# schmeing/ReSeq

Measured on AMD Instinct MI355X. Metric: simulated read-pairs/sec (2x150 bp), higher is better.
Workload: dtype f64

## Files before the change

### reseq_amd/csrc/rsq_format.h

```cpp
#pragma once
#include "rsq_reads.h"

namespace rsq {

#if RSQ_DEVICE_BUILD
#ifndef RSQ_BIN_KEYS_LDS
#define RSQ_BIN_KEYS_LDS 4096
#endif
constexpr uint32_t kBinKeysLds = RSQ_BIN_KEYS_LDS;
constexpr uint32_t kBinItemsPerThread = 16, kBinBlock = 256;

__device__ inline void bin_count_key(uint32_t key, bool valid, uint32_t n_keys, uint32_t *hist, uint32_t *s_hist) {
    if (n_keys <= kBinKeysLds) {
        for (uint32_t k = threadIdx.x; k < n_keys; k += blockDim.x) s_hist[k] = 0;
        __syncthreads();
        if (valid) atomicAdd(&s_hist[key], 1u);
        __syncthreads();
        for (uint32_t k = threadIdx.x; k < n_keys; k += blockDim.x)
            if (s_hist[k]) atomicAdd(&hist[k], s_hist[k]);
    } else if (valid) atomicAdd(&hist[key], 1u);
}
__global__ void __launch_bounds__(kBinBlock) k_pair_tiles(DevSim S, const Fragment *frags, const FragmentVar *fvars, uint64_t n_pairs, uint64_t adapter_only_first, uint16_t *key_of,
                                                         uint32_t *hist) {
    __shared__ uint32_t s_hist[kBinKeysLds];
    const uint64_t pair = (uint64_t)blockIdx.x * blockDim.x + threadIdx.x;
    const bool valid = pair < n_pairs;
    uint32_t key = 0;
    if (valid) {
        Fragment f{};
        if (frags) f = frags[pair];
        const PairStream ps = pair_stream(frags ? &f : nullptr, fvars ? fvars[pair].sub : 0u, adapter_only_first + pair);
        key = draw_tile(S, ps.c0, ps.c1, ps.c2, pair_c3(kDomPair, ps.strand, 2, f.allele));
        key_of[pair] = (uint16_t)key;
    }
    bin_count_key(key, valid, S.n_tiles, hist, s_hist);
}
__global__ void __launch_bounds__(kBinBlock) k_record_tiles(DevSim S, const uint8_t *segs, uint64_t first_index, uint64_t n, uint16_t *key_of, uint32_t *hist) {
    __shared__ uint32_t s_hist[kBinKeysLds];
    const uint64_t i = (uint64_t)blockIdx.x * blockDim.x + threadIdx.x;
    const bool valid = i < n;
    uint32_t key = 0;
    if (valid) {
        const uint64_t idx = first_index + i;
        key = (segs[i] ? S.n_tiles : 0u) + draw_tile(S, (uint32_t)idx, (uint32_t)(idx >> 32), 0u, pair_c3(kDomErrModel, 0, 2));
        key_of[i] = (uint16_t)key;
    }
    bin_count_key(key, valid, 2u * S.n_tiles, hist, s_hist);
}
__global__ void __launch_bounds__(1024) k_bins_plan(const uint32_t *hist, uint32_t n_keys, uint32_t n_bins, uint32_t *bin_first, uint32_t *bin_count, uint32_t *cursor,
                                                    uint32_t *chunk_ptr, uint32_t *next_chunk, uint32_t *workers) {
    __shared__ uint32_t s_part[1024], s_chunks[1024];
    const uint32_t t = threadIdx.x, per = (n_bins + 1023u) / 1024u, lo = t * per < n_bins ? t * per : n_bins, hi = lo + per < n_bins ? lo + per : n_bins;
    uint32_t items = 0, chunks = 0;
    for (uint32_t b = lo; b < hi; ++b) {
        const uint32_t c = hist[b % n_keys];
        if (b < n_keys) items += c;
        chunks += (c + 63u) / 64u;
    }
    s_part[t] = items;
    s_chunks[t] = chunks;
    __syncthreads();
    for (uint32_t d = 1; d < 1024u; d <<= 1) {
        const uint32_t a = t >= d ? s_part[t - d] : 0u, c = t >= d ? s_chunks[t - d] : 0u;
        __syncthreads();
        s_part[t] += a;
        s_chunks[t] += c;
        __syncthreads();
    }
    uint32_t at = s_part[t] - items, chunk_at = s_chunks[t] - chunks;
    for (uint32_t b = lo; b < hi; ++b) {
        const uint32_t c = hist[b % n_keys];
        if (b < n_keys) {
            cursor[b] = at;
            for (uint32_t r = b; r < n_bins; r += n_keys) bin_first[r] = at, bin_count[r] = c;
            at += c;
        }
        chunk_ptr[b] = chunk_at;
        chunk_at += (c + 63u) / 64u;
        next_chunk[b] = workers[b] = 0;
    }
    if (t == 1023u) chunk_ptr[n_bins] = s_chunks[1023];
}
__global__ void __launch_bounds__(kBinBlock) k_bin_scatter(const uint16_t *key_of, uint64_t n, uint32_t n_keys, uint32_t *cursor, uint32_t *perm, const Fragment *frags,
                                                          const FragmentVar *fvars, Fragment *frags_sorted, FragmentVar *fvars_sorted) {
    __shared__ uint32_t s_count[kBinKeysLds], s_base[kBinKeysLds];
    const uint64_t first = (uint64_t)blockIdx.x * (kBinBlock * kBinItemsPerThread);
    auto place = [&](uint32_t at, uint64_t i) {
        perm[at] = (uint32_t)i;
        if (frags) frags_sorted[at] = frags[i];
        if (fvars) fvars_sorted[at] = fvars[i];
    };
    if (n_keys > kBinKeysLds) {
        for (uint32_t j = 0; j < kBinItemsPerThread; ++j) {
            const uint64_t i = first + (uint64_t)j * kBinBlock + threadIdx.x;
            if (i < n) place(atomicAdd(&cursor[key_of[i]], 1u), i);
        }
        return;
    }
    for (uint32_t k = threadIdx.x; k < n_keys; k += kBinBlock) s_count[k] = 0;
    __syncthreads();
    uint32_t rank[kBinItemsPerThread], key[kBinItemsPerThread];
#pragma unroll
    for (uint32_t j = 0; j < kBinItemsPerThread; ++j) {
        const uint64_t i = first + (uint64_t)j * kBinBlock + threadIdx.x;
        key[j] = i < n ? key_of[i] : 0xFFFFFFFFu;
        rank[j] = i < n ? atomicAdd(&s_count[key[j]], 1u) : 0u;
    }
    __syncthreads();
    for (uint32_t k = threadIdx.x; k < n_keys; k += kBinBlock)
        if (s_count[k]) s_base[k] = atomicAdd(&cursor[k], s_count[k]);
    __syncthreads();
#pragma unroll
    for (uint32_t j = 0; j < kBinItemsPerThread; ++j)
        if (key[j] != 0xFFFFFFFFu) place(s_base[key[j]] + rank[j], first + (uint64_t)j * kBinBlock + threadIdx.x);
}

struct FragmentRange {
    uint32_t lo[2], hi[2];
};
__global__ void k_fragment_range(const uint8_t *segs, const uint32_t *frag_len, uint64_t n, FragmentRange range, uint32_t *first_bad) {
    const uint64_t i = (uint64_t)blockIdx.x * blockDim.x + threadIdx.x;
    if (i >= n) return;
    const uint32_t seg = segs[i] ? 1u : 0u, fl = frag_len[i];
    if (fl < range.lo[seg] || fl >= range.hi[seg]) atomicMin(first_bad, (uint32_t)i);
}
__global__ void k_record_flags(const uint8_t *segs, uint64_t n, uint32_t *flags) {
    const uint64_t i = (uint64_t)blockIdx.x * blockDim.x + threadIdx.x;
    if (i < n) flags[i] = segs[i] ? 1u : 0u;
}
__global__ void k_record_partition(const uint8_t *segs, uint64_t n, const uint64_t *ones_before, uint32_t *rec_index, uint32_t *rec_count) {
    const uint64_t i = (uint64_t)blockIdx.x * blockDim.x + threadIdx.x;
    const uint32_t n1 = (uint32_t)ones_before[n], n0 = (uint32_t)n - n1;
    if (i == 0) {
        rec_count[0] = n0;
        rec_count[1] = n1;
    }
    if (i >= n) return;
    const uint32_t before = (uint32_t)ones_before[i];
    if (segs[i]) rec_index[n0 + before] = (uint32_t)i;
    else rec_index[(uint32_t)i - before] = (uint32_t)i;
}

__global__ void __launch_bounds__(256) k_methylation_templates(DevSim S, const Fragment *frags, uint64_t n_pairs, RawLayout raw) {
    const uint64_t r = (uint64_t)blockIdx.x * blockDim.x + threadIdx.x;
    if (r >= 2u * n_pairs) return;
    const uint32_t seg = r >= n_pairs ? 1u : 0u;
    convert_template(S, frags[r - seg * n_pairs], seg, raw.templates + r * raw.template_words, raw.template_words);
}

__global__ void __launch_bounds__(256) k_variant_templates(DevSim S, const Fragment *frags, const FragmentVar *fvars, uint64_t n_pairs, RawLayout raw) {
    const uint64_t r = (uint64_t)blockIdx.x * blockDim.x + threadIdx.x;
    if (r >= 2u * n_pairs) return;
    const uint32_t seg = r >= n_pairs ? 1u : 0u;
    const uint64_t pair = r - seg * n_pairs;
    variant_template(S, frags[pair], fvars[pair], seg, raw.templates + r * raw.template_words, raw.template_words);
}

template <bool PERM, uint32_t ITEMS>
struct WaveImage {
    const uint64_t *offsets;
    char *dst;
    uint32_t lane, skew, bytes, slot_at;
    uint64_t row, item, g_begin;
    bool active, through_lds;
    static __device__ __forceinline__ uint64_t first() { return (uint64_t)blockIdx.x * ITEMS; }
    __device__ __forceinline__ WaveImage(const uint64_t *offsets, uint64_t n, char *dst, uint32_t lds_bytes, const uint32_t *perm, uint32_t lane) : offsets(offsets), dst(dst), lane(lane) {
        const uint64_t last = first() + ITEMS < n ? first() + ITEMS : n;
        row = first() + (lane & (ITEMS - 1u));
        active = row < last;
        item = PERM ? (active ? perm[row] : 0u) : row;
        g_begin = PERM ? (active ? offsets[item] : 0u) : offsets[first()];
        const uint64_t g_end = PERM ? (active ? offsets[item + 1u] : 0u) : offsets[last];
        skew = (uint32_t)((uint64_t)(uintptr_t)(dst + g_begin) & 15u);
        bytes = (uint32_t)(g_end - g_begin);
        const uint32_t slot = (lds_bytes / ITEMS) & ~15u;
        through_lds = PERM ? __all(skew + bytes <= slot) != 0 : skew + bytes <= lds_bytes;
        slot_at = PERM ? (lane & (ITEMS - 1u)) * slot : 0u;
    }
    __device__ __forceinline__ RSQ_LDS char *item_text(char *image) const { return (RSQ_LDS char *)image + slot_at + skew + (PERM ? 0u : (uint32_t)(offsets[item] - g_begin)); }
    __device__ __forceinline__ void store_out(const char *image) const {
        __syncthreads();
        const uint32_t lo = skew, hi = skew + bytes;
        char *g_chunk0 = dst + g_begin - skew;
        const char *s_from = image + slot_at;
        for (uint32_t c = (PERM ? lane / ITEMS : lane) * 16u; c < hi; c += (PERM ? 64u / ITEMS : 64u) * 16u) {
            if (c >= lo && c + 16u <= hi) {
                *reinterpret_cast<uint4 *>(g_chunk0 + c) = *reinterpret_cast<const uint4 *>(s_from + c);
            } else {
                for (uint32_t b = c < lo ? lo : c; b < c + 16u && b < hi; ++b) g_chunk0[b] = s_from[b];
            }
        }
    }
};

#ifndef RSQ_FORMAT_RECORDS
#define RSQ_FORMAT_RECORDS 16
#endif
constexpr uint32_t kFormatRecords = RSQ_FORMAT_RECORDS, kFormatLdsMax = 16u * 1024u, kFormatLdsMin = 1024u;
RSQ_HD uint32_t format_lds_bytes(uint64_t record_bytes, bool slots) {
    const uint64_t want = (kFormatRecords * record_bytes + 16u + 127u) & ~(uint64_t)127u;
    const uint32_t image = (uint32_t)(want < kFormatLdsMin ? kFormatLdsMin : want > kFormatLdsMax ? kFormatLdsMax : want);
    return !slots ? image : image + 16u * kFormatRecords < kFormatLdsMax ? image + 16u * kFormatRecords : kFormatLdsMax;
}
__global__ void __launch_bounds__(256) k_max_size(const uint32_t *sizes, uint64_t n, uint32_t *longest) {
    uint32_t m = 0;
    for (uint64_t i = (uint64_t)blockIdx.x * blockDim.x + threadIdx.x; i < n; i += (uint64_t)gridDim.x * blockDim.x) m = max(m, sizes[i]);
    for (uint32_t d = 32; d; d >>= 1) m = max(m, (uint32_t)__shfl_xor((int)m, (int)d, 64));
    if ((threadIdx.x & 63u) == 0 && m) atomicMax(longest, m);
}
template <bool PERM>
__global__ void __launch_bounds__(64) k_format_write(DevSim S, NameTable names, const Fragment *frags, uint64_t n_pairs, uint64_t adapter_only_first, RawLayout raw,
                                                    const uint64_t *offsets0, const uint64_t *offsets1, char *dst0, char *dst1, uint64_t cap0, uint64_t cap1,
                                                    const FragmentVar *fvars, const uint32_t *perm, uint32_t lds_bytes) {
    extern __shared__ __attribute__((aligned(16))) char s_text[];
    using Image = WaveImage<PERM, kFormatRecords>;
    const uint32_t lane = threadIdx.x, seg = blockIdx.y, part = lane / kFormatRecords;
    constexpr uint32_t kLineParts = 32u / kFormatRecords;
    const bool is_qual = part >= kLineParts;
    const uint32_t sub = part % kLineParts;
    if (Image::first() >= n_pairs) return;
    const uint64_t *offsets = seg ? offsets1 : offsets0;
    char *dst = seg ? dst1 : dst0;
    if (offsets[n_pairs] > (seg ? cap1 : cap0)) return;
    const Image im(offsets, n_pairs, dst, lds_bytes, perm, lane);
    const uint64_t pair = im.item;
    ReadMeta m;
    Fragment f;
    FragmentVar fv;
    uint64_t r = 0;
    if (im.active) {
        r = (uint64_t)seg * n_pairs + im.row;
        m = raw.meta[r];
        if (frags) f = frags[pair];
        if (frags && fvars) fv = fvars[pair];
    }
    const WordColumn seq = raw.seq_of(r), qual = raw.qual_of(r), ops = raw.ops_of(r);
    const uint64_t ao_number = adapter_only_first + pair + 1u;
    if (!im.through_lds) {
        if (im.active && part == 0u) format_record(S, names, frags != nullptr, f, ao_number, m, seq, qual, ops, dst + offsets[pair], frags && fvars, fv);
        return;
    }
    if (im.active) {
        const uint32_t header = (uint32_t)(offsets[pair + 1u] - offsets[pair]) - 2u * m.read_len - 4u;
        const uint32_t all_words = (m.read_len + 3u) >> 2, per = (all_words + kLineParts - 1u) / kLineParts;
        const uint32_t first_word = sub * per, line_at = header + (is_qual ? m.read_len + 3u : 0u);
        const uint32_t part_at = part == 0u ? 0u : line_at + (4u * first_word < m.read_len ? 4u * first_word : m.read_len);
        WordSinkT<RSQ_LDS char *> t(im.item_text(s_text) + part_at);
        if (part == 0u) format_header(S, names, frags != nullptr, f, ao_number, m, ops, t, frags && fvars, fv);
        format_line_part(is_qual ? qual : seq, m.read_len, is_qual, first_word, per, sub == kLineParts - 1u, t);
        t.finish();
    }
    im.store_out(s_text);
}

RSQ_HD uint32_t error_model_record_size(const ReadMeta &m, uint32_t id_len) { return 1u + id_len + 1u + m.cigar_chars + 2u + digits_u32(m.num_errors) + 1u + 2u * m.read_len + 4u; }
struct RecordIds {
    const char *chars;
    const uint64_t *off;
    const uint32_t *at, *len;
    RSQ_HD const char *begin(uint64_t i) const { return chars + (off ? off[i] : (uint64_t)at[i] + 1u); }
    RSQ_HD uint32_t length(uint64_t i) const { return off ? (uint32_t)(off[i + 1] - off[i]) : len[i]; }
};
__global__ void __launch_bounds__(256) k_record_text_sizes(RawLayout raw, uint64_t n, RecordIds ids, uint32_t *sizes) {
    const uint64_t row = (uint64_t)blockIdx.x * blockDim.x + threadIdx.x;
    if (row >= n) return;
    const uint64_t i = raw.item_of(row);
    sizes[i] = error_model_record_size(raw.meta[row], ids.length(i));
}
template <bool PERM>
__global__ void __launch_bounds__(64) k_record_text_waves(RawLayout raw, uint64_t n, RecordIds ids, const uint64_t *offsets, char *dst, uint64_t cap, uint32_t lds_bytes) {
    extern __shared__ __attribute__((aligned(16))) char s_text[];
    using Image = WaveImage<PERM, kFormatRecords>;
    constexpr uint32_t kLineParts = 32u / kFormatRecords;
    const uint32_t lane = threadIdx.x, part = lane / kFormatRecords, sub = part % kLineParts;
    const bool is_qual = part >= kLineParts;
    if (Image::first() >= n || offsets[n] > cap) return;
    const Image im(offsets, n, dst, lds_bytes, raw.order, lane);
    const uint64_t row = im.row, item = im.item;
    const bool active = im.active;
    ReadMeta m{};
    if (active) m = raw.meta[row];
    const WordColumn seq = raw.seq_of(active ? row : 0u), qual = raw.qual_of(active ? row : 0u), ops = raw.ops_of(active ? row : 0u);
    auto header = [&](auto &t) {
        t.ch('@');
        t.str(ids.begin(item), ids.length(item));
        t.ch(' ');
        cigar_replay(ops, m, t);
        t.str(" E", 2);
        t.num((uint32_t)m.num_errors);
        t.ch('\n');
    };
    if (!im.through_lds) {
        if (active && part == 0u) {
            WordSinkT<char *> t(dst + offsets[item]);
            header(t);
            format_line(seq, m.read_len, false, t);
            format_line(qual, m.read_len, true, t);
            t.finish();
        }
        return;
    }
    if (active) {
        const uint32_t head = (uint32_t)(offsets[item + 1u] - offsets[item]) - 2u * m.read_len - 4u;
        const uint32_t all_words = (m.read_len + 3u) >> 2, per = (all_words + kLineParts - 1u) / kLineParts, first_word = sub * per;
        const uint32_t line_at = head + (is_qual ? m.read_len + 3u : 0u), part_at = part == 0u ? 0u : line_at + (4u * first_word < m.read_len ? 4u * first_word : m.read_len);
        WordSinkT<RSQ_LDS char *> t(im.item_text(s_text) + part_at);
        if (part == 0u) header(t);
        format_line_part(is_qual ? qual : seq, m.read_len, is_qual, first_word, per, sub == kLineParts - 1u, t);
        t.finish();
    }
    im.store_out(s_text);
}

#endif

}
```

### reseq_amd/csrc/rsq_sam.h

```cpp
#pragma once
#include "rsq_format.h"

namespace rsq {

struct SamMate {
    uint16_t q, t;
    uint16_t lead, trail;
    uint16_t cigar_chars;
    uint16_t pad;
    uint32_t bytes;
};
static_assert(sizeof(SamMate) == 16, "two mates are one 32-byte load");
struct SamPair {
    SamMate mate[2];
};

RSQ_HD uint32_t sam_op_at(const WordColumn &ops, uint32_t it) { return (ops.at(it >> 4) >> ((it & 15u) * 2u)) & 3u; }

RSQ_HD SamMate sam_walk(const WordColumn &ops, const ReadMeta &m) {
    SamMate w{};
    const uint32_t n = m.n_iter_m;
    uint32_t chars = 0;
    if (m.plain) {
        w.q = w.t = (uint16_t)n;
        if (n) chars = digits_u32(n) + 1u;
    } else {
        uint32_t q = 0, t = 0, run = 0, cur = 3u, runs = 0;
        auto flush = [&](bool last) {
            if (!run) return;
            if (cur == 1u && runs == 1u) w.lead = (uint16_t)run;
            else if (cur == 1u && last) w.trail = (uint16_t)run;
            else chars += digits_u32(run) + 1u;
        };
        for (uint32_t it = 0; it < n; ++it) {
            if (!(it & 15u) && it + 16u <= n && !ops.at(it >> 4)) {
                if (cur != 0u) {
                    flush(false);
                    cur = 0u;
                    run = 0;
                    ++runs;
                }
                run += 16u;
                q += 16u;
                t += 16u;
                it += 15u;
                continue;
            }
            const uint32_t c = sam_op_at(ops, it);
            if (c != cur) {
                flush(false);
                cur = c;
                run = 0;
                ++runs;
            }
            ++run;
            q += c != 1u;
            t += c != 2u;
        }
        flush(true);
        w.q = (uint16_t)q;
        w.t = (uint16_t)t;
    }
    const uint32_t clip = (uint32_t)m.read_len - w.q;
    if (clip) chars += digits_u32(clip) + 1u;
    w.cigar_chars = (uint16_t)(chars ? chars : 1u);
    return w;
}

template <class Sink>
RSQ_HD void sam_cigar(const WordColumn &ops, const ReadMeta &m, const SamMate &w, bool reverse, Sink &t) {
    const uint32_t clip = (uint32_t)m.read_len - w.q;
    bool any = false;
    if (reverse && clip) {
        t.element('S', clip);
        any = true;
    }
    if (m.plain) {
        if (m.n_iter_m) {
            t.element('M', m.n_iter_m);
            any = true;
        }
    } else {
        const uint32_t lo = w.lead, hi = (uint32_t)m.n_iter_m - w.trail;
        uint32_t cur = 3u, run = 0;
        for (uint32_t i = lo; i < hi; ++i) {
            const uint32_t it = reverse ? hi - 1u - (i - lo) : i;
            if ((reverse ? (it & 15u) == 15u && it >= lo + 15u : !(it & 15u) && it + 16u <= hi) && (cur == 0u || !run) && !ops.at(it >> 4)) {
                cur = 0u;
                run += 16u;
                i += 15u;
                continue;
            }
            const uint32_t c = sam_op_at(ops, it);
            if (c != cur) {
                if (run) t.element(cur == 0u ? 'M' : cur == 1u ? 'D' : 'I', run);
                cur = c;
                run = 0;
            }
            ++run;
        }
        if (run) {
            t.element(cur == 0u ? 'M' : cur == 1u ? 'D' : 'I', run);
            any = true;
        }
    }
    if (!reverse && clip) {
        t.element('S', clip);
        any = true;
    }
    if (!any) t.ch('*');
}

struct SamAlign {
    uint32_t flag, pos, pnext;
    int32_t tlen;
    uint32_t mapped, reverse;
};
RSQ_HD SamAlign sam_align(bool has_f, const Fragment &f, uint32_t seg, const SamMate &w0, const SamMate &w1) {
    SamAlign a{};
    if (!has_f || !f.len) {
        a.flag = seg ? 141u : 77u;
        return a;
    }
    const uint32_t end = f.start + f.len;
    int32_t pos[2], last[2];
    for (uint32_t s = 0; s < 2u; ++s) {
        const SamMate &w = s ? w1 : w0;
        const bool rev = s != f.strand;
        const uint32_t d_left = rev ? w.trail : w.lead, d_right = rev ? w.lead : w.trail;
        pos[s] = (int32_t)((rev ? end - w.t : f.start) + 1u + d_left);
        last[s] = pos[s] + (int32_t)((uint32_t)w.t - d_left - d_right) - 1;
    }
    const uint32_t o = seg ^ 1u;
    const bool rev = seg != f.strand;
    a.mapped = 1u;
    a.reverse = rev ? 1u : 0u;
    a.flag = 0x1u | 0x2u | (rev ? 0x10u : 0x20u) | (seg ? 0x80u : 0x40u);
    a.pos = (uint32_t)pos[seg];
    a.pnext = (uint32_t)pos[o];
    const int32_t span = (last[0] > last[1] ? last[0] : last[1]) - (pos[0] < pos[1] ? pos[0] : pos[1]) + 1;
    const bool leftmost = pos[seg] < pos[o] || (pos[seg] == pos[o] && seg == 0u);
    a.tlen = leftmost ? span : -span;
    return a;
}

template <class Sink>
RSQ_HD void sam_qname(const DevSim &S, const NameTable &names, bool has_f, const Fragment &f, uint64_t adapter_only_number, const ReadMeta &m, Sink &t) {
    t.str(names.base_identifier, names.base_len);
    if (has_f) {
        const uint32_t end = f.start + f.len;
        t.num(f.block);
        t.ch('_');
        t.num(f.number);
        t.ch(':');
        t.num(f.strand ? end : f.start + 1u);
        t.ch(':');
        t.str(names.names + names.name_ptr[f.seq], names.name_ptr[f.seq + 1] - names.name_ptr[f.seq]);
        t.ch(':');
        t.num(f.strand ? f.start + 1u : end);
    } else {
        t.ch('0');
        t.ch('_');
        t.num(adapter_only_number);
        t.str(":0:Adapter:0", 12);
    }
    t.ch(':');
    t.num((uint32_t)S.tiles[m.tile_id]);
    t.str(":1337:1337", 10);
}
RSQ_HD uint32_t sam_qname_size(const DevSim &S, const NameTable &names, bool has_f, const Fragment &f, uint64_t adapter_only_number, const ReadMeta &m) {
    uint32_t n = names.base_len + 1u + digits_u32(S.tiles[m.tile_id]) + 10u;
    if (has_f) {
        const uint32_t end = f.start + f.len;
        n += digits_u32(f.block) + 1u + digits_u32(f.number) + 1u + digits_u32(f.start + 1u) + 1u + (names.name_ptr[f.seq + 1] - names.name_ptr[f.seq]) + 1u + digits_u32(end);
    } else n += 2u + digits_u64(adapter_only_number) + 12u;
    return n;
}
RSQ_HD uint32_t sam_tlen_chars(int32_t v) { return v < 0 ? 1u + digits_u32((uint32_t)-(int64_t)v) : digits_u32((uint32_t)v); }

template <class Sink>
RSQ_HD void sam_head(const DevSim &S, const NameTable &names, bool has_f, const Fragment &f, uint64_t adapter_only_number, const ReadMeta &m, const WordColumn &ops, const SamMate &w,
                     const SamAlign &a, Sink &t) {
    sam_qname(S, names, has_f, f, adapter_only_number, m, t);
    t.ch('\t');
    t.num(a.flag);
    t.ch('\t');
    if (a.mapped) {
        t.str(names.names + names.name_ptr[f.seq], names.name_ptr[f.seq + 1] - names.name_ptr[f.seq]);
        t.ch('\t');
        t.num(a.pos);
        t.str("\t60\t", 4);
        sam_cigar(ops, m, w, a.reverse != 0u, t);
        t.str("\t=\t", 3);
        t.num(a.pnext);
        t.ch('\t');
        if (a.tlen < 0) {
            t.ch('-');
            t.num((uint32_t)-(int64_t)a.tlen);
        } else t.num((uint32_t)a.tlen);
        t.ch('\t');
    } else t.str("*\t0\t0\t*\t*\t0\t0\t", 14);
}
RSQ_HD uint32_t sam_head_size(const DevSim &S, const NameTable &names, bool has_f, const Fragment &f, uint64_t adapter_only_number, const ReadMeta &m, const SamMate &w, const SamAlign &a) {
    uint32_t n = sam_qname_size(S, names, has_f, f, adapter_only_number, m) + 1u + digits_u32(a.flag) + 1u;
    if (a.mapped)
        n += (names.name_ptr[f.seq + 1] - names.name_ptr[f.seq]) + 1u + digits_u32(a.pos) + 4u + w.cigar_chars + 3u + digits_u32(a.pnext) + 1u + sam_tlen_chars(a.tlen) + 1u;
    else n += 14u;
    return n;
}
RSQ_HD uint32_t sam_byte_reverse(uint32_t w) {
#if defined(__HIP_DEVICE_COMPILE__)
    return __builtin_amdgcn_perm(0u, w, 0x00010203u);
#else
    return (w >> 24) | ((w >> 8) & 0xFF00u) | ((w << 8) & 0xFF0000u) | (w << 24);
#endif
}
RSQ_HD uint32_t sam_complement_letters(uint32_t codes) {
#if defined(__HIP_DEVICE_COMPILE__)
    return __builtin_amdgcn_perm(0x4E4E4E4Eu, 0x41434754u, codes);
#else
    uint32_t out = 0;
    for (uint32_t k = 0; k < 4u; ++k) {
        const uint32_t b = (codes >> (8u * k)) & 0xFFu;
        out |= (uint32_t)("TGCAN"[b < 4u ? b : 4u]) << (8u * k);
    }
    return out;
#endif
}
RSQ_HD uint32_t sam_funnel(uint32_t hi, uint32_t lo, uint32_t bytes) {
#if defined(__HIP_DEVICE_COMPILE__)
    return __builtin_amdgcn_alignbyte(hi, lo, bytes);
#else
    return (uint32_t)((((uint64_t)hi << 32) | lo) >> (8u * bytes));
#endif
}
template <class Sink>
RSQ_HD void sam_line(const WordColumn &row, uint32_t read_len, bool is_qual, bool reverse, uint32_t phred_offset, Sink &t) {
    const uint32_t words = (read_len + 3u) >> 2, odd = read_len & 3u;
    const uint32_t shift = ((phred_offset - 33u) & 0xFFu) * 0x01010101u;
    constexpr uint32_t kAhead = 10u;
    for (uint32_t i = 0; i < words; i += kAhead) {
        uint32_t w[kAhead + 1u];
#pragma unroll
        for (uint32_t k = 0; k <= kAhead; ++k) {
            const uint32_t j = i + k;
            w[k] = j < words && (k < kAhead || (reverse && odd)) ? row.at(reverse ? words - 1u - j : j) : 0u;
        }
#pragma unroll
        for (uint32_t k = 0; k < kAhead; ++k) {
            if (i + k >= words) break;
            uint32_t v = w[k];
            if (reverse) v = sam_byte_reverse(odd ? sam_funnel(w[k], w[k + 1u], odd) : v);
            const uint32_t text = is_qual ? v - shift : reverse ? sam_complement_letters(v) : base_letters(v), left = read_len - 4u * (i + k);
            t.bytes(text, left < 4u ? left : 4u);
        }
    }
}
template <class Sink>
RSQ_HD void sam_tags(const ReadMeta &m, const WordColumn &ops, Sink &t) {
    t.str("\tXC:Z:", 6);
    cigar_replay(ops, m, t);
    t.str("\tXE:i:", 6);
    t.num((uint32_t)m.num_errors);
    t.ch('\n');
}
RSQ_HD uint32_t sam_tags_size(const ReadMeta &m) { return 6u + m.cigar_chars + 6u + digits_u32(m.num_errors) + 1u; }

RSQ_HD uint32_t sam_record_size(const DevSim &S, const NameTable &names, bool has_f, const Fragment &f, uint64_t adapter_only_number, const ReadMeta &m, const SamMate &w,
                                const SamAlign &a) {
    return sam_head_size(S, names, has_f, f, adapter_only_number, m, w, a) + 2u * m.read_len + 1u + sam_tags_size(m);
}
template <class P>
RSQ_HD uint32_t sam_record(const DevSim &S, const NameTable &names, bool has_f, const Fragment &f, uint64_t adapter_only_number, const ReadMeta &m, const WordColumn &seq,
                           const WordColumn &qual, const WordColumn &ops, const SamMate &w, const SamAlign &a, P dst) {
    WordSinkT<P> t(dst);
    sam_head(S, names, has_f, f, adapter_only_number, m, ops, w, a, t);
    sam_line(seq, m.read_len, false, a.reverse != 0u, S.phred_offset, t);
    t.ch('\t');
    sam_line(qual, m.read_len, true, a.reverse != 0u, S.phred_offset, t);
    sam_tags(m, ops, t);
    t.finish();
    return t.n;
}

#if RSQ_DEVICE_BUILD
__global__ void __launch_bounds__(256) k_sam_sizes(DevSim S, NameTable names, const Fragment *frags, uint64_t n_pairs, uint64_t adapter_only_first, RawLayout raw, const uint32_t *perm,
                                                   SamPair *side, uint32_t *sizes) {
    const uint64_t row = (uint64_t)blockIdx.x * blockDim.x + threadIdx.x;
    if (row >= n_pairs) return;
    const uint64_t pair = perm ? perm[row] : row;
    Fragment f{};
    if (frags) f = frags[pair];
    const ReadMeta m0 = raw.meta[row], m1 = raw.meta[n_pairs + row];
    SamPair p;
    p.mate[0] = sam_walk(raw.ops_of(row), m0);
    p.mate[1] = sam_walk(raw.ops_of(n_pairs + row), m1);
    const uint64_t ao_number = adapter_only_first + pair + 1u;
    p.mate[0].bytes = sam_record_size(S, names, frags != nullptr, f, ao_number, m0, p.mate[0], sam_align(frags != nullptr, f, 0u, p.mate[0], p.mate[1]));
    p.mate[1].bytes = sam_record_size(S, names, frags != nullptr, f, ao_number, m1, p.mate[1], sam_align(frags != nullptr, f, 1u, p.mate[0], p.mate[1]));
    side[row] = p;
    sizes[pair] = p.mate[0].bytes + p.mate[1].bytes;
}

constexpr uint32_t kSamPairs = 16, kSamLdsMax = 32u * 1024u, kSamLdsMin = 2048u;
RSQ_HD uint32_t sam_lds_bytes(uint64_t pair_bytes, bool slots) {
    const uint64_t want = (kSamPairs * (pair_bytes + (slots ? 16u : 0u)) + 16u + 127u) & ~(uint64_t)127u;
    return (uint32_t)(want < kSamLdsMin ? kSamLdsMin : want > kSamLdsMax ? kSamLdsMax : want);
}
template <bool PERM>
__global__ void __launch_bounds__(64) k_sam_write(DevSim S, NameTable names, const Fragment *frags, uint64_t n_pairs, uint64_t adapter_only_first, RawLayout raw, const SamPair *side,
                                                 const uint64_t *offsets, char *dst, uint64_t cap, const uint64_t *fastq_end0, const uint64_t *fastq_end1, uint64_t fastq_cap0,
                                                 uint64_t fastq_cap1, const uint32_t *perm, uint32_t lds_bytes) {
    extern __shared__ __attribute__((aligned(16))) char s_sam[];
    using Image = WaveImage<PERM, kSamPairs>;
    const uint32_t lane = threadIdx.x, part = lane / kSamPairs, seg = part >> 1, half = part & 1u;
    if (Image::first() >= n_pairs) return;
    if (offsets[n_pairs] > cap || *fastq_end0 > fastq_cap0 || *fastq_end1 > fastq_cap1) return;
    const Image im(offsets, n_pairs, dst, lds_bytes, perm, lane);
    const uint64_t pair = im.item;
    ReadMeta m{};
    Fragment f{};
    SamPair p{};
    uint64_t r = 0;
    if (im.active) {
        r = (uint64_t)seg * n_pairs + im.row;
        m = raw.meta[r];
        p = side[im.row];
        if (frags) f = frags[pair];
    }
    const bool has_f = frags != nullptr;
    const WordColumn seq = raw.seq_of(r), qual = raw.qual_of(r), ops = raw.ops_of(r);
    const uint64_t ao_number = adapter_only_first + pair + 1u;
    const SamMate w = seg ? p.mate[1] : p.mate[0];
    const SamAlign a = sam_align(has_f, f, seg, p.mate[0], p.mate[1]);
    const uint32_t rec_at = seg ? p.mate[0].bytes : 0u;
    if (!im.through_lds) {
        if (im.active && half == 0u) sam_record(S, names, has_f, f, ao_number, m, seq, qual, ops, w, a, dst + offsets[pair] + rec_at);
        return;
    }
    if (im.active) {
        const uint32_t qual_at = w.bytes - sam_tags_size(m) - m.read_len;
        WordSinkT<RSQ_LDS char *> t(im.item_text(s_sam) + rec_at + (half ? qual_at : 0u));
        if (half == 0u) {
            sam_head(S, names, has_f, f, ao_number, m, ops, w, a, t);
            sam_line(seq, m.read_len, false, a.reverse != 0u, S.phred_offset, t);
            t.ch('\t');
        } else {
            sam_line(qual, m.read_len, true, a.reverse != 0u, S.phred_offset, t);
            sam_tags(m, ops, t);
        }
        t.finish();
    }
    im.store_out(s_sam);
}
#endif

}
```

Measured before the change: 231.8 million.

## Assemble LDS text images with word-wise atomic ORs into zero-cleared LDS

```diff
diff --git a/reseq_amd/csrc/rsq_format.h b/reseq_amd/csrc/rsq_format.h
--- a/reseq_amd/csrc/rsq_format.h
+++ b/reseq_amd/csrc/rsq_format.h
@@ -1,7 +1,254 @@
 #pragma once
+#include <string.h>
+
 #include "rsq_reads.h"
 
 namespace rsq {
+
+RSQ_HD void image_or(RSQ_LDS uint32_t *w, uint32_t v) {
+#if defined(__HIP_DEVICE_COMPILE__)
+    __hip_atomic_fetch_or(w, v, __ATOMIC_RELAXED, __HIP_MEMORY_SCOPE_WORKGROUP);
+#else
+    uint32_t x;
+    memcpy(&x, w, 4);
+    x |= v;
+    memcpy(w, &x, 4);
+#endif
+}
+RSQ_HD uint32_t image_bytes_at(uint32_t hi, uint32_t lo, uint32_t at) {
+#if defined(__HIP_DEVICE_COMPILE__)
+    return __builtin_amdgcn_perm(hi, lo, 0x03020100u + at * 0x01010101u);
+#else
+    return (uint32_t)((((uint64_t)hi << 32) | lo) >> (8u * at));
+#endif
+}
+RSQ_HD uint32_t image_word(const uint32_t *p) {
+#if defined(__HIP_DEVICE_COMPILE__)
+    return *p;
+#else
+    uint32_t x;
+    memcpy(&x, p, 4);
+    return x;
+#endif
+}
+RSQ_HD bool image_any(bool p) {
+#if defined(__HIP_DEVICE_COMPILE__)
+    return __any(p) != 0;
+#else
+    return p;
+#endif
+}
+RSQ_HD constexpr uint32_t chars4(char a, char b = 0, char c = 0, char d = 0) {
+    return (uint32_t)(uint8_t)a | ((uint32_t)(uint8_t)b << 8) | ((uint32_t)(uint8_t)c << 16) | ((uint32_t)(uint8_t)d << 24);
+}
+RSQ_HD uint32_t four_digits(uint32_t g) {
+    const uint32_t q = (g * 5243u) >> 19, r = g - 100u * q;
+    const uint32_t x = q | (r << 16);
+    const uint32_t t = ((x * 103u) >> 10) & 0x000F000Fu;
+    const uint32_t u = x - 10u * t;
+    return (t | (u << 8)) + 0x30303030u;
+}
+RSQ_HD uint32_t count_digits4(uint32_t g) { return 1u + (g >= 10u) + (g >= 100u) + (g >= 1000u); }
+
+struct ImageSink {
+    RSQ_LDS uint32_t *w;
+    uint32_t lo;
+    uint32_t pending, n;
+    RSQ_HD explicit ImageSink(RSQ_LDS char *dst)
+        : w(reinterpret_cast<RSQ_LDS uint32_t *>(dst - ((uint32_t)(uintptr_t)dst & 3u))), lo(0), pending((uint32_t)(uintptr_t)dst & 3u), n(0) {}
+    RSQ_HD void push(uint32_t bytes, uint32_t count) {
+        const uint64_t wide = (uint64_t)bytes << (8u * pending);
+        lo |= (uint32_t)wide;
+        pending += count;
+        n += count;
+        const bool full = pending >= 4u;
+        if (full) image_or(w, lo);
+        lo = full ? (uint32_t)(wide >> 32) : lo;
+        w += full ? 1 : 0;
+        pending &= 3u;
+    }
+    RSQ_HD void push4(uint32_t bytes) {
+        const uint64_t wide = (uint64_t)bytes << (8u * pending);
+        image_or(w, lo | (uint32_t)wide);
+        lo = (uint32_t)(wide >> 32);
+        w += 1;
+        n += 4u;
+    }
+    RSQ_HD void finish() {
+        if (pending) image_or(w, lo);
+    }
+    RSQ_HD void ch(char c) { push((uint8_t)c, 1u); }
+    RSQ_HD void bytes(uint32_t word, uint32_t count) { push(count < 4u ? word & ((1u << (8u * count)) - 1u) : word, count); }
+    RSQ_HD void str(const char *s, uint32_t len, uint32_t head = 0, uint32_t tail = 0) {
+        if (__builtin_constant_p(len) && __builtin_constant_p(s[0]) && !head && !tail) {
+            uint32_t i = 0;
+            for (; i + 4u <= len; i += 4u) push4(chars4(s[i], s[i + 1u], s[i + 2u], s[i + 3u]));
+            if (i < len) {
+                uint32_t word = 0;
+                for (uint32_t k = 0; i + k < len; ++k) word |= (uint32_t)(uint8_t)s[i + k] << (8u * k);
+                push(word, len - i);
+            }
+            return;
+        }
+        const uint32_t a = (uint32_t)(uintptr_t)s & 3u;
+        words(reinterpret_cast<const uint32_t *>(s - a), a, len, head, tail);
+    }
+    RSQ_HD void words(const uint32_t *from, uint32_t a, uint32_t len, uint32_t head = 0, uint32_t tail = 0) {
+        uint32_t low = 0, next = 0;
+        if (len) low = image_word(from + next++);
+        if (head) {
+            if (a) {
+                --a;
+                low = (low & ~(0xFFu << (8u * a))) | (head << (8u * a));
+            } else {
+                a = 3u;
+                next = 0;
+                low = head << 24;
+            }
+            ++len;
+        }
+        uint32_t i = 0;
+        for (; i + 4u <= len; i += 4u, ++next) {
+            const uint32_t high = a + len > i + 4u ? image_word(from + next) : 0u;
+            push4(image_bytes_at(high, low, a));
+            low = high;
+        }
+        uint32_t rest = len - i;
+        const uint32_t high = a + len > i + 4u ? image_word(from + next) : 0u;
+        uint32_t word = image_bytes_at(high, low, a) & ((1u << (8u * rest)) - 1u);
+        if (tail) {
+            word |= tail << (8u * rest);
+            ++rest;
+        }
+        push(word, rest);
+    }
+    RSQ_HD void num(uint32_t v, uint32_t tail = 0, uint32_t tail_len = 0) {
+        if (!image_any(v >= 10000u)) {
+            const uint32_t digits = count_digits4(v), total = digits + tail_len, at = 4u - digits;
+            push(image_bytes_at(tail, four_digits(v), at), total < 4u ? total : 4u);
+            if (image_any(total > 4u)) push(tail >> (8u * at), total > 4u ? total - 4u : 0u);
+            return;
+        }
+        const uint32_t upper = v / 10000u, hi = upper / 10000u, mid = upper - 10000u * hi;
+        const uint32_t top = hi ? hi : upper ? mid : v, digits = (hi ? 8u : upper ? 4u : 0u) + count_digits4(top);
+        const uint32_t x[4] = {four_digits(hi), four_digits(mid), four_digits(v - 10000u * upper), tail};
+        const uint32_t skip = 12u - digits, sw = skip >> 2, at = skip & 3u, total = digits + tail_len;
+        const uint32_t x0 = sw == 0u ? x[0] : sw == 1u ? x[1] : x[2], x1 = sw == 0u ? x[1] : sw == 1u ? x[2] : x[3], x2 = sw == 0u ? x[2] : sw == 1u ? x[3] : 0u, x3 = sw == 0u ? x[3] : 0u;
+        push(image_bytes_at(x1, x0, at), total < 4u ? total : 4u);
+        push(image_bytes_at(x2, x1, at), total < 4u ? 0u : total < 8u ? total - 4u : 4u);
+        if (image_any(total > 8u)) push(image_bytes_at(x3, x2, at), total < 8u ? 0u : total < 12u ? total - 8u : 4u);
+        if (image_any(total > 12u)) push(x3 >> (8u * at), total < 12u ? 0u : total - 12u);
+    }
+    RSQ_HD void nine_digits(uint32_t v) {
+        const uint32_t upper = v / 10000u, hi = upper / 10000u;
+        push('0' + hi, 1u);
+        push4(four_digits(upper - 10000u * hi));
+        push4(four_digits(v - 10000u * upper));
+    }
+    RSQ_HD void num(uint64_t v, uint32_t tail = 0, uint32_t tail_len = 0) {
+        if (v <= 0xFFFFFFFFull) return num((uint32_t)v, tail, tail_len);
+        const uint64_t kE9 = 1000000000ull, upper = v / kE9;
+        if (upper >= kE9) {
+            num((uint32_t)(upper / kE9));
+            nine_digits((uint32_t)(upper % kE9));
+        } else num((uint32_t)upper);
+        nine_digits((uint32_t)(v % kE9));
+        push(tail, tail_len);
+    }
+    RSQ_HD void element(char op, uint32_t count) { num(count, (uint8_t)op, 1u); }
+};
+
+RSQ_HD void image_header(const DevSim &S, const NameTable &names, bool has_f, const Fragment &f, uint64_t adapter_only_number, const ReadMeta &m, const WordColumn &ops, ImageSink &t,
+                         bool has_fv, const FragmentVar &fv) {
+    t.words(reinterpret_cast<const uint32_t *>(names.base_identifier), 0u, names.base_len, '@');
+    if (has_f) {
+        const uint32_t end = has_fv ? fv.end : f.start + f.len;
+        t.num(f.block, '_', 1u);
+        if (1u < S.num_alleles) {
+            t.num(f.number, chars4('_', 'a', 'l', 'l'), 4u);
+            t.push(chars4('e', 'l', 'e'), 3u);
+            t.num((uint32_t)f.allele, ':', 1u);
+        } else t.num(f.number, ':', 1u);
+        t.num(f.strand ? end : f.start + 1u, ':', 1u);
+        t.str(names.names + names.name_ptr[f.seq], names.name_ptr[f.seq + 1] - names.name_ptr[f.seq], 0u, ':');
+        t.num(f.strand ? f.start + 1u : end, ':', 1u);
+    } else {
+        t.push(chars4('0', '_'), 2u);
+        t.num(adapter_only_number, chars4(':', '0', ':', 'A'), 4u);
+        t.push4(chars4('d', 'a', 'p', 't'));
+        t.push4(chars4('e', 'r', ':', '0'));
+        t.push(':', 1u);
+    }
+    t.num((uint32_t)S.tiles[m.tile_id], chars4(':', '1', '3', '3'), 4u);
+    t.push4(chars4('7', ':', '1', '3'));
+    t.push(chars4('3', '7', ' '), 3u);
+    cigar_replay(ops, m, t);
+    t.push(chars4(' ', 'E'), 2u);
+    t.num((uint32_t)m.num_errors, '\n', 1u);
+}
+
+RSQ_HD void image_line_part(const WordColumn &row, uint32_t read_len, bool is_qual, uint32_t first_word, uint32_t n_words, bool with_end, RSQ_LDS char *dst) {
+    const uint32_t begin = 4u * first_word < read_len ? 4u * first_word : read_len, left = read_len - begin;
+    const uint32_t n_bytes = left < 4u * n_words ? left : 4u * n_words, full = n_bytes >> 2, rest = n_bytes & 3u;
+    const uint32_t phase = (uint32_t)(uintptr_t)dst & 3u, at = 4u - phase;
+    RSQ_LDS uint32_t *out = reinterpret_cast<RSQ_LDS uint32_t *>(dst - phase);
+    constexpr uint32_t kAhead = 10u;
+    uint32_t before = 0;
+    for (uint32_t i = 0; i < full; i += kAhead) {
+        uint32_t w[kAhead];
+        if (i + kAhead <= full) {
+#pragma unroll
+            for (uint32_t k = 0; k < kAhead; ++k) w[k] = row.at(first_word + i + k);
+#pragma unroll
+            for (uint32_t k = 0; k < kAhead; ++k) {
+                const uint32_t text = is_qual ? w[k] : base_letters(w[k]);
+                image_or(out + i + k, image_bytes_at(text, before, at));
+                before = text;
+            }
+        } else {
+#pragma unroll
+            for (uint32_t k = 0; k < kAhead; ++k) w[k] = i + k < full ? row.at(first_word + i + k) : 0u;
+#pragma unroll
+            for (uint32_t k = 0; k < kAhead; ++k) {
+                if (i + k < full) {
+                    const uint32_t text = is_qual ? w[k] : base_letters(w[k]);
+                    image_or(out + i + k, image_bytes_at(text, before, at));
+                    before = text;
+                }
+            }
+        }
+    }
+    uint64_t x = with_end ? (is_qual ? (uint64_t)'\n' : (uint64_t)chars4('\n', '+', '\n')) : 0u;
+    const uint32_t used = phase + rest + (with_end ? (is_qual ? 1u : 3u) : 0u);
+    x <<= 8u * rest;
+    if (rest) {
+        const uint32_t last = row.at(first_word + full);
+        x |= (is_qual ? last : base_letters(last)) & ((1u << (8u * rest)) - 1u);
+    }
+    const uint32_t x0 = (uint32_t)x, x1 = (uint32_t)(x >> 32);
+    if (used > 0u) image_or(out + full, image_bytes_at(x0, before, at));
+    if (used > 4u) image_or(out + full + 1u, image_bytes_at(x1, x0, at));
+    if (used > 8u) image_or(out + full + 2u, image_bytes_at(0u, x1, at));
+}
+
+#ifndef RSQ_FORMAT_RECORDS
+#define RSQ_FORMAT_RECORDS 16
+#endif
+constexpr uint32_t kFormatRecords = RSQ_FORMAT_RECORDS, kFormatLineParts = 32u / kFormatRecords;
+template <class Head>
+RSQ_HD void image_record_part(const ReadMeta &m, const WordColumn &seq, const WordColumn &qual, uint32_t head_bytes, uint32_t part, RSQ_LDS char *text, Head &&head) {
+    const bool is_qual = part >= kFormatLineParts;
+    const uint32_t sub = part % kFormatLineParts;
+    const uint32_t all_words = ((uint32_t)m.read_len + 3u) >> 2, per = (all_words + kFormatLineParts - 1u) / kFormatLineParts;
+    const uint32_t first_word = sub * per, line_at = head_bytes + (is_qual ? m.read_len + 3u : 0u);
+    RSQ_LDS char *at = text + line_at + (4u * first_word < m.read_len ? 4u * first_word : m.read_len);
+    if (part == 0u) {
+        ImageSink t(text);
+        head(t);
+        t.finish();
+    }
+    image_line_part(is_qual ? qual : seq, m.read_len, is_qual, first_word, per, sub == kFormatLineParts - 1u, at);
+}
 
 #if RSQ_DEVICE_BUILD
 #ifndef RSQ_BIN_KEYS_LDS
@@ -178,6 +425,10 @@
         slot_at = PERM ? (lane & (ITEMS - 1u)) * slot : 0u;
     }
     __device__ __forceinline__ RSQ_LDS char *item_text(char *image) const { return (RSQ_LDS char *)image + slot_at + skew + (PERM ? 0u : (uint32_t)(offsets[item] - g_begin)); }
+    __device__ __forceinline__ void clear(char *image, uint32_t lds_bytes) const {
+        for (uint32_t c = lane * 16u; c < lds_bytes; c += 64u * 16u) *reinterpret_cast<uint4 *>(image + c) = uint4{0u, 0u, 0u, 0u};
+        __syncthreads();
+    }
     __device__ __forceinline__ void store_out(const char *image) const {
         __syncthreads();
         const uint32_t lo = skew, hi = skew + bytes;
@@ -193,10 +444,7 @@
     }
 };
 
-#ifndef RSQ_FORMAT_RECORDS
-#define RSQ_FORMAT_RECORDS 16
-#endif
-constexpr uint32_t kFormatRecords = RSQ_FORMAT_RECORDS, kFormatLdsMax = 16u * 1024u, kFormatLdsMin = 1024u;
+constexpr uint32_t kFormatLdsMax = 16u * 1024u, kFormatLdsMin = 1024u;
 RSQ_HD uint32_t format_lds_bytes(uint64_t record_bytes, bool slots) {
     const uint64_t want = (kFormatRecords * record_bytes + 16u + 127u) & ~(uint64_t)127u;
     const uint32_t image = (uint32_t)(want < kFormatLdsMin ? kFormatLdsMin : want > kFormatLdsMax ? kFormatLdsMax : want);
@@ -215,9 +463,6 @@
     extern __shared__ __attribute__((aligned(16))) char s_text[];
     using Image = WaveImage<PERM, kFormatRecords>;
     const uint32_t lane = threadIdx.x, seg = blockIdx.y, part = lane / kFormatRecords;
-    constexpr uint32_t kLineParts = 32u / kFormatRecords;
-    const bool is_qual = part >= kLineParts;
-    const uint32_t sub = part % kLineParts;
     if (Image::first() >= n_pairs) return;
     const uint64_t *offsets = seg ? offsets1 : offsets0;
     char *dst = seg ? dst1 : dst0;
@@ -240,15 +485,10 @@
         if (im.active && part == 0u) format_record(S, names, frags != nullptr, f, ao_number, m, seq, qual, ops, dst + offsets[pair], frags && fvars, fv);
         return;
     }
+    im.clear(s_text, lds_bytes);
     if (im.active) {
         const uint32_t header = (uint32_t)(offsets[pair + 1u] - offsets[pair]) - 2u * m.read_len - 4u;
-        const uint32_t all_words = (m.read_len + 3u) >> 2, per = (all_words + kLineParts - 1u) / kLineParts;
-        const uint32_t first_word = sub * per, line_at = header + (is_qual ? m.read_len + 3u : 0u);
-        const uint32_t part_at = part == 0u ? 0u : line_at + (4u * first_word < m.read_len ? 4u * first_word : m.read_len);
-        WordSinkT<RSQ_LDS char *> t(im.item_text(s_text) + part_at);
-        if (part == 0u) format_header(S, names, frags != nullptr, f, ao_number, m, ops, t, frags && fvars, fv);
-        format_line_part(is_qual ? qual : seq, m.read_len, is_qual, first_word, per, sub == kLineParts - 1u, t);
-        t.finish();
+        image_record_part(m, seq, qual, header, part, im.item_text(s_text), [&](ImageSink &t) { image_header(S, names, frags != nullptr, f, ao_number, m, ops, t, frags && fvars, fv); });
     }
     im.store_out(s_text);
 }
@@ -271,9 +511,7 @@
 __global__ void __launch_bounds__(64) k_record_text_waves(RawLayout raw, uint64_t n, RecordIds ids, const uint64_t *offsets, char *dst, uint64_t cap, uint32_t lds_bytes) {
     extern __shared__ __attribute__((aligned(16))) char s_text[];
     using Image = WaveImage<PERM, kFormatRecords>;
-    constexpr uint32_t kLineParts = 32u / kFormatRecords;
-    const uint32_t lane = threadIdx.x, part = lane / kFormatRecords, sub = part % kLineParts;
-    const bool is_qual = part >= kLineParts;
+    const uint32_t lane = threadIdx.x, part = lane / kFormatRecords;
     if (Image::first() >= n || offsets[n] > cap) return;
     const Image im(offsets, n, dst, lds_bytes, raw.order, lane);
     const uint64_t row = im.row, item = im.item;
@@ -290,6 +528,12 @@
         t.num((uint32_t)m.num_errors);
         t.ch('\n');
     };
+    auto image_head = [&](ImageSink &t) {
+        t.str(ids.begin(item), ids.length(item), '@', ' ');
+        cigar_replay(ops, m, t);
+        t.push(chars4(' ', 'E'), 2u);
+        t.num((uint32_t)m.num_errors, '\n', 1u);
+    };
     if (!im.through_lds) {
         if (active && part == 0u) {
             WordSinkT<char *> t(dst + offsets[item]);
@@ -300,14 +544,10 @@
         }
         return;
     }
+    im.clear(s_text, lds_bytes);
     if (active) {
         const uint32_t head = (uint32_t)(offsets[item + 1u] - offsets[item]) - 2u * m.read_len - 4u;
-        const uint32_t all_words = (m.read_len + 3u) >> 2, per = (all_words + kLineParts - 1u) / kLineParts, first_word = sub * per;
-        const uint32_t line_at = head + (is_qual ? m.read_len + 3u : 0u), part_at = part == 0u ? 0u : line_at + (4u * first_word < m.read_len ? 4u * first_word : m.read_len);
-        WordSinkT<RSQ_LDS char *> t(im.item_text(s_text) + part_at);
-        if (part == 0u) header(t);
-        format_line_part(is_qual ? qual : seq, m.read_len, is_qual, first_word, per, sub == kLineParts - 1u, t);
-        t.finish();
+        image_record_part(m, seq, qual, head, part, im.item_text(s_text), image_head);
     }
     im.store_out(s_text);
 }
diff --git a/reseq_amd/csrc/rsq_sam.h b/reseq_amd/csrc/rsq_sam.h
--- a/reseq_amd/csrc/rsq_sam.h
+++ b/reseq_amd/csrc/rsq_sam.h
@@ -338,9 +338,10 @@
         if (im.active && half == 0u) sam_record(S, names, has_f, f, ao_number, m, seq, qual, ops, w, a, dst + offsets[pair] + rec_at);
         return;
     }
+    im.clear(s_sam, lds_bytes);
     if (im.active) {
         const uint32_t qual_at = w.bytes - sam_tags_size(m) - m.read_len;
-        WordSinkT<RSQ_LDS char *> t(im.item_text(s_sam) + rec_at + (half ? qual_at : 0u));
+        ImageSink t(im.item_text(s_sam) + rec_at + (half ? qual_at : 0u));
         if (half == 0u) {
             sam_head(S, names, has_f, f, ao_number, m, ops, w, a, t);
             sam_line(seq, m.read_len, false, a.reverse != 0u, S.phred_offset, t);
```

Measured after the change: 235.5 million, median of 6. 1.02x the previous value.
